# chengstone/cchess-zero

Hardware: AMD Instinct MI355X
Metric: MCTS simulations/sec (whole node), playout=1600, 7-block net (higher is better)
Workload: dtype mx6

## Files before the change

cchess_zero_amd/csrc/cz_trunk_mx.h:

```cpp
#pragma once
#include "cz_conv_kernel.h"

namespace czconv {

#include "cz_trunk_mx_asm.inc"

struct MXGeo {
    static constexpr int P = 2;
    static constexpr int ROWS = P * 90;
    static constexpr int THREADS = 512;
    static constexpr int ENT = 224;
    static constexpr int XPLANE = ENT * 16, YPLANE = ENT * 8, SPLANE = ENT * 4;
    static constexpr int X_OFF = 0, Y_OFF = 8 * XPLANE, S_OFF = Y_OFF + 8 * YPLANE;
    static constexpr int HI_OFF = S_OFF + 2 * SPLANE;
    static constexpr int ZERO_OFF = HI_OFF + ROWS * CV_ROWB;
    static constexpr int W_OFF = ZERO_OFF + CV_ROWB;
    static constexpr int SLAB_BYTES = 16384;
    static constexpr int SLAB_SHIFT = 14;
    static constexpr int SLABS_PER_LAYER = 36;
    static constexpr int LDS_BYTES = W_OFF + TW_NBUF * SLAB_BYTES;
    static constexpr int PLANES_OFF = W_OFF + 3 * SLAB_BYTES;
    static constexpr int HEADW_OFF = LDS_BYTES;
    static constexpr int LDS_TOTAL = LDS_BYTES + 3 * 128 * 4;
    static constexpr int F32_ROWB = 512;
// ... 198 lines not shown
    }

#define MX_OPERANDS(NAB, NKEY)                                                                                       \
            : [c0] "+v"(acc[0]), [c1] "+v"(acc[1]), [c2] "+v"(acc[2]),                                                 \
              [a0h0] "+v"(fa.a[0]), [a0h1] "+v"(fa.a[1]), [a0h2] "+v"(fa.a[2]), [w0] "+v"(fa.w),                      \
              [a1h0] "+v"(fb.a[0]), [a1h1] "+v"(fb.a[1]), [a1h2] "+v"(fb.a[2]), [w1] "+v"(fb.w),                      \
              [sb0] "+v"(sb[0]), [sb1] "+v"(sb[1]), [sb2] "+v"(sb[2]),                                                \
              [t0] "=&v"(t0), [t1] "=&v"(t1), [t2] "=&v"(t2), [ws] "=&v"(wsr), [keep] "=&s"(keep)                      \
            : [ab0] "v"(ab[0]), [ab1] "v"(ab[1]), [ab2] "v"(ab[2]), [key0] "v"(key[0]), [key1] "v"(key[1]),            \
              [key2] "v"(key[2]), [nab0] "v"(NAB[0]), [nab1] "v"(NAB[1]), [nab2] "v"(NAB[2]), [nkey0] "v"(NKEY[0]),     \
              [nkey1] "v"(NKEY[1]), [nkey2] "v"(NKEY[2]), [xr0] "v"(xr[0]), [xr1] "v"(xr[1]), [xr2] "v"(xr[2]),        \
              [yr0] "v"(yr[0]), [yr1] "v"(yr[1]), [yr2] "v"(yr[2]), [vb] "v"(vb), [vy] "v"(vy), [vs] "v"(vs),          \
              [vbn] "v"(vbn), [voff0] "v"(voff0), [voff1] "v"(voff1), [sbase] "s"(sbase), [ldst] "s"(ldst)
#define MX_CLOBBERS "memory", "scc", "v232", "v233", "v234", "v235", "v236", "v237", "v238", "v239", "v240", "v241", "v242", "v243", \
                    "v244", "v245", "v246", "v247", "v248", "v249", "v250", "v251", "v252", "v253", "v254", "v255"
#define MX_ARGS()                                                                                                    \
            TRUNK_SLAB_ARGS(wpk, const int vy = vy0 + slot; const int vs = vs0 + slot;)
#define MX_RUN(ASMSTR, NAB, NKEY)                                                                                    \
        {                                                                                                            \
            MX_ARGS()                                                                                                \
            asm volatile(ASMSTR MX_OPERANDS(NAB, NKEY) : MX_CLOBBERS);                                               \
            ++g;                                                                                                     \
        }
#define MX_RUNV(ASMSTR, NAB, NKEY)                           \
        {                                                                                                            \
            MX_ARGS()                                                                                                \
            asm volatile(ASMSTR MX_OPERANDS(NAB, NKEY), [skipm] "s"(skipm) : MX_CLOBBERS, "vcc");                    \
            ++g;                                                                                                     \
        }

#ifdef MX_TIMING
    unsigned long long tm_loop = 0, tm_epi = 0, tm_set = 0, tm_t0 = __builtin_readcyclecounter();
    const unsigned long long tm_first = tm_t0 - clk_c0;
#define MX_TM(acc) { const unsigned long long n_ = __builtin_readcyclecounter(); acc += n_ - tm_t0; tm_t0 = n_; }
#else
#define MX_TM(acc)
#endif
    struct MxFrag { bf16x8 a[3], w; };
    int g = 0;
    int skipm;
    asm volatile("s_cmp_lt_u32 %1, 4\n\ts_cselect_b32 %0, 1, 0" : "=s"(skipm) : "s"(wave_u) : "scc");
#pragma unroll 1
    for (int layer = 0; layer < nlayers; ++layer) {
        f32x16 acc[3];
        init_acc(acc, nullptr, (layer & 1) != 0);
        int ab[3], key[3], nab[3], nkey[3], xr[3], yr[3], nxr[3], nyr[3], t0, t1, t2, wsr;
        int sb[3] = {0, 0, 0};
        MxFrag fa, fb;
        tap_addr(0, ab, key, xr, yr);
        {
            const int vb = vb0 + (((unsigned)g & 3u) << Geo::SLAB_SHIFT);
#pragma unroll
            for (int i = 0; i < 3; ++i) {
                fa.a[i] = *reinterpret_cast<const bf16x8 *>(smem + ab[i] + ((0 ^ key[i]) << 4));
                fb.a[i] = *reinterpret_cast<const bf16x8 *>(smem + ab[i] + ((2 ^ key[i]) << 4));
            }
            fa.w = *reinterpret_cast<const bf16x8 *>(smem + vb);
            fb.w = *reinterpret_cast<const bf16x8 *>(smem + vb + 4096);
            asm volatile("" : "+v"(fa.a[0]), "+v"(fa.a[1]), "+v"(fa.a[2]), "+v"(fa.w), "+v"(fb.a[0]), "+v"(fb.a[1]), "+v"(fb.a[2]), "+v"(fb.w));
        }
        MX_TM(tm_set)
        int tap = 0;
#pragma unroll 1
        for (; tap < 3; ++tap) {
            MX_RUNV(MX_SKIP0_ASM_Q0, ab, key)
            MX_RUNV(MX_SKIP0_ASM_Q1, ab, key)
            MX_RUNV(MX_SKIP0_ASM_Q2, ab, key)
            tap_addr(tap + 1, nab, nkey, nxr, nyr);
            MX_RUNV(MX_SKIP0_ASM_Q3, nab, nkey)
#pragma unroll
            for (int i = 0; i < 3; ++i) { ab[i] = nab[i]; key[i] = nkey[i]; xr[i] = nxr[i]; yr[i] = nyr[i]; }
        }
#pragma unroll 1
        for (; tap < 8; ++tap) {
            MX_RUN(MX_SLAB_ASM_Q0, ab, key)
            MX_RUN(MX_SLAB_ASM_Q1, ab, key)
            MX_RUN(MX_SLAB_ASM_Q2, ab, key)
            tap_addr(tap + 1, nab, nkey, nxr, nyr);
            MX_RUN(MX_SLAB_ASM_Q3, nab, nkey)
#pragma unroll
            for (int i = 0; i < 3; ++i) { ab[i] = nab[i]; key[i] = nkey[i]; xr[i] = nxr[i]; yr[i] = nyr[i]; }
        }
        MX_RUN(MX_SLAB_ASM_Q0, ab, key)
        MX_RUN(MX_SLAB_ASM_Q1, ab, key)
        MX_RUN(MX_SLAB_ASM_Q2, ab, key)
        MX_RUN(MX_SLAB_ASM_Q3_LAST, ab, key)
        const bool last = layer + 1 == nlayers;
        if (last) asm volatile("s_waitcnt vmcnt(0)" ::: "memory");
        else load_bias(bias + (layer + 1) * 128);
        asm volatile("s_nop 15\n\ts_nop 15\n\ts_nop 15" ::: "memory");
        MX_TM(tm_loop)
        refresh_rk();
// ... 27 lines not shown
        for (int r = tid; r < nrows; r += Geo::THREADS) {
            const int k = lds_row_of(r);
            float acc0 = 0.f, acc1 = 0.f, acc2 = 0.f;
#pragma unroll 4
            for (int c = 0; c < 32; ++c) {
                const float4 e = *reinterpret_cast<const float4 *>(smem + k * Geo::F32_ROWB + ((c ^ (k & 31)) << 4));
                const float *w0_ = hw + c * 4, *w1_ = hw + 128 + c * 4, *w2_ = hw + 256 + c * 4;
                acc0 += e.x * w0_[0] + e.y * w0_[1] + e.z * w0_[2] + e.w * w0_[3];
                acc1 += e.x * w1_[0] + e.y * w1_[1] + e.z * w1_[2] + e.w * w1_[3];
                acc2 += e.x * w2_[0] + e.y * w2_[1] + e.z * w2_[2] + e.w * w2_[3];
            }
            float *o = head_out + ((size_t)pos0 * 90 + r) * 3;
            o[0] = fmaxf(acc0 + head_b[0], 0.f);
            o[1] = fmaxf(acc1 + head_b[1], 0.f);
            o[2] = fmaxf(acc2 + head_b[2], 0.f);
        }
    }
}
#undef MX_OPERANDS
#undef MX_CLOBBERS
#undef MX_ARGS
#undef MX_RUN
#undef MX_RUNV

}
```

cchess_zero_amd/csrc/cz_trunk_mx_asm.inc:

```
#define MX_SLAB_ASM_Q0 \
    "s_mov_b32 %[keep], m0\n\t" \
    "s_waitcnt lgkmcnt(4)\n\t" \
    "v_mfma_f32_32x32x16_f16 %[c0], %[w0], %[a0h0], %[c0]\n\t" \
    "ds_read_b128 v[232:235], %[xr0] offset:0\n\t" \
    "ds_read_b64 v[236:237], %[yr0] offset:28672\n\t" \
    "ds_read_b128 v[238:241], %[xr1] offset:0\n\t" \
    "ds_read_b64 v[242:243], %[yr1] offset:28672\n\t" \
    "v_lshrrev_b32 %[t0], 1, %[yr0]\n\t" \
    "v_lshrrev_b32 %[t1], 1, %[yr1]\n\t" \
    "v_lshrrev_b32 %[t2], 1, %[yr2]\n\t" \
    "v_mfma_f32_32x32x16_f16 %[c1], %[w0], %[a0h1], %[c1]\n\t" \
    "ds_read_b128 v[244:247], %[xr2] offset:0\n\t" \
    "ds_read_b64 v[248:249], %[yr2] offset:28672\n\t" \
    "ds_read_b32 %[sb0], %[t0] offset:43008\n\t" \
    "ds_read_b32 %[sb1], %[t1] offset:43008\n\t" \
    "ds_read_b32 %[sb2], %[t2] offset:43008\n\t" \
    "v_mfma_f32_32x32x16_f16 %[c2], %[w0], %[a0h2], %[c2]\n\t" \
    "ds_read_b128 v[250:253], %[vb] offset:8192\n\t" \
    "ds_read_b64 v[254:255], %[vy]\n\t" \
    "ds_read_b32 %[ws], %[vs]\n\t" \
    "s_waitcnt vmcnt(2)\n\t" \
    "s_barrier\n\t" \
    "s_waitcnt lgkmcnt(12)\n\t" \
    "v_mfma_f32_32x32x16_f16 %[c0], %[w1], %[a1h0], %[c0]\n\t" \
// ... 170 lines not shown
    "ds_read_b128 %[w0], %[vbn]\n\t" \
    "s_waitcnt lgkmcnt(4)\n\t" \
    "v_mfma_scale_f32_32x32x64_f8f6f4 %[c0], v[250:255], v[232:237], %[c0], %[ws], %[sb0] op_sel:[0,1,0] op_sel_hi:[0,1,0] cbsz:2 blgp:2\n\t" \
    "v_xor_b32 %[t0], 2, %[nkey0]\n\t" \
    "v_xor_b32 %[t1], 2, %[nkey1]\n\t" \
    "v_xor_b32 %[t2], 2, %[nkey2]\n\t" \
    "v_lshl_add_u32 %[t0], %[t0], 4, %[nab0]\n\t" \
    "v_lshl_add_u32 %[t1], %[t1], 4, %[nab1]\n\t" \
    "v_lshl_add_u32 %[t2], %[t2], 4, %[nab2]\n\t" \
    "s_mov_b32 m0, %[ldst]\n\t" \
    "s_nop 0\n\t" \
    "global_load_lds_dwordx4 %[voff0], %[sbase]\n\t" \
    "v_mfma_scale_f32_32x32x64_f8f6f4 %[c1], v[250:255], v[238:243], %[c1], %[ws], %[sb1] op_sel:[0,1,0] op_sel_hi:[0,1,0] cbsz:2 blgp:2\n\t" \
    "ds_read_b128 %[a1h0], %[t0]\n\t" \
    "ds_read_b128 %[a1h1], %[t1]\n\t" \
    "s_add_u32 m0, %[ldst], 0x2000\n\t" \
    "s_nop 0\n\t" \
    "global_load_lds_dwordx4 %[voff1], %[sbase]\n\t" \
    "v_mfma_scale_f32_32x32x64_f8f6f4 %[c2], v[250:255], v[244:249], %[c2], %[ws], %[sb2] op_sel:[0,1,0] op_sel_hi:[0,1,0] cbsz:2 blgp:2\n\t" \
    "ds_read_b128 %[a1h2], %[t2]\n\t" \
    "ds_read_b128 %[w1], %[vbn] offset:4096\n\t" \
    "s_mov_b32 m0, %[keep]\n\t"

#define MX_SKIP0_ASM_Q0 \
    "s_cmp_lg_u32 %[skipm], 0\n\t" \
    "s_cselect_b64 vcc, -1, 0\n\t" \
    "s_mov_b32 %[keep], m0\n\t" \
    "s_waitcnt lgkmcnt(4)\n\t" \
    "s_cbranch_vccnz 1f\n\t" \
    "v_mfma_f32_32x32x16_f16 %[c0], %[w0], %[a0h0], %[c0]\n\t" \
    "1:\n\t" \
    "ds_read_b128 v[232:235], %[xr0] offset:0\n\t" \
    "ds_read_b64 v[236:237], %[yr0] offset:28672\n\t" \
    "ds_read_b128 v[238:241], %[xr1] offset:0\n\t" \
    "ds_read_b64 v[242:243], %[yr1] offset:28672\n\t" \
    "v_lshrrev_b32 %[t0], 1, %[yr0]\n\t" \
    "v_lshrrev_b32 %[t1], 1, %[yr1]\n\t" \
    "v_lshrrev_b32 %[t2], 1, %[yr2]\n\t" \
    "v_mfma_f32_32x32x16_f16 %[c1], %[w0], %[a0h1], %[c1]\n\t" \
    "ds_read_b128 v[244:247], %[xr2] offset:0\n\t" \
    "ds_read_b64 v[248:249], %[yr2] offset:28672\n\t" \
    "ds_read_b32 %[sb0], %[t0] offset:43008\n\t" \
    "ds_read_b32 %[sb1], %[t1] offset:43008\n\t" \
    "ds_read_b32 %[sb2], %[t2] offset:43008\n\t" \
    "v_mfma_f32_32x32x16_f16 %[c2], %[w0], %[a0h2], %[c2]\n\t" \
    "ds_read_b128 v[250:253], %[vb] offset:8192\n\t" \
    "ds_read_b64 v[254:255], %[vy]\n\t" \
    "ds_read_b32 %[ws], %[vs]\n\t" \
    "s_waitcnt vmcnt(2)\n\t" \
    "s_barrier\n\t" \
    "s_waitcnt lgkmcnt(12)\n\t" \
    "s_cbranch_vccnz 1f\n\t" \
    "v_mfma_f32_32x32x16_f16 %[c0], %[w1], %[a1h0], %[c0]\n\t" \
    "1:\n\t" \
    "v_xor_b32 %[t0], 4, %[key0]\n\t" \
    "v_xor_b32 %[t1], 4, %[key1]\n\t" \
    "v_xor_b32 %[t2], 4, %[key2]\n\t" \
    "v_lshl_add_u32 %[t0], %[t0], 4, %[ab0]\n\t" \
    "v_lshl_add_u32 %[t1], %[t1], 4, %[ab1]\n\t" \
    "v_lshl_add_u32 %[t2], %[t2], 4, %[ab2]\n\t" \
    "v_mfma_f32_32x32x16_f16 %[c1], %[w1], %[a1h1], %[c1]\n\t" \
    "ds_read_b128 %[a0h0], %[t0]\n\t" \
    "ds_read_b128 %[a0h1], %[t1]\n\t" \
    "v_mfma_f32_32x32x16_f16 %[c2], %[w1], %[a1h2], %[c2]\n\t" \
    "ds_read_b128 %[a0h2], %[t2]\n\t" \
    "ds_read_b128 %[w0], %[vbn]\n\t" \
    "s_waitcnt lgkmcnt(4)\n\t" \
    "s_cbranch_vccnz 1f\n\t" \
    "v_mfma_scale_f32_32x32x64_f8f6f4 %[c0], v[250:255], v[232:237], %[c0], %[ws], %[sb0] op_sel:[0,0,0] op_sel_hi:[0,0,0] cbsz:2 blgp:2\n\t" \
    "1:\n\t" \
    "v_xor_b32 %[t0], 6, %[key0]\n\t" \
    "v_xor_b32 %[t1], 6, %[key1]\n\t" \
    "v_xor_b32 %[t2], 6, %[key2]\n\t" \
    "v_lshl_add_u32 %[t0], %[t0], 4, %[ab0]\n\t" \
    "v_lshl_add_u32 %[t1], %[t1], 4, %[ab1]\n\t" \
    "v_lshl_add_u32 %[t2], %[t2], 4, %[ab2]\n\t" \
    "s_mov_b32 m0, %[ldst]\n\t" \
    "s_nop 0\n\t" \
    "global_load_lds_dwordx4 %[voff0], %[sbase]\n\t" \
    "v_mfma_scale_f32_32x32x64_f8f6f4 %[c1], v[250:255], v[238:243], %[c1], %[ws], %[sb1] op_sel:[0,0,0] op_sel_hi:[0,0,0] cbsz:2 blgp:2\n\t" \
    "ds_read_b128 %[a1h0], %[t0]\n\t" \
    "ds_read_b128 %[a1h1], %[t1]\n\t" \
    "s_add_u32 m0, %[ldst], 0x2000\n\t" \
    "s_nop 0\n\t" \
    "global_load_lds_dwordx4 %[voff1], %[sbase]\n\t" \
    "v_mfma_scale_f32_32x32x64_f8f6f4 %[c2], v[250:255], v[244:249], %[c2], %[ws], %[sb2] op_sel:[0,0,0] op_sel_hi:[0,0,0] cbsz:2 blgp:2\n\t" \
    "ds_read_b128 %[a1h2], %[t2]\n\t" \
    "ds_read_b128 %[w1], %[vbn] offset:4096\n\t" \
    "s_mov_b32 m0, %[keep]\n\t"

#define MX_SKIP0_ASM_Q1 \
    "s_cmp_lg_u32 %[skipm], 0\n\t" \
    "s_cselect_b64 vcc, -1, 0\n\t" \
    "s_mov_b32 %[keep], m0\n\t" \
    "s_waitcnt lgkmcnt(4)\n\t" \
    "s_cbranch_vccnz 1f\n\t" \
    "v_mfma_f32_32x32x16_f16 %[c0], %[w0], %[a0h0], %[c0]\n\t" \
    "1:\n\t" \
    "ds_read_b128 v[232:235], %[xr0] offset:7168\n\t" \
    "ds_read_b64 v[236:237], %[yr0] offset:32256\n\t" \
    "ds_read_b128 v[238:241], %[xr1] offset:7168\n\t" \
    "ds_read_b64 v[242:243], %[yr1] offset:32256\n\t" \
    "v_mfma_f32_32x32x16_f16 %[c1], %[w0], %[a0h1], %[c1]\n\t" \
    "ds_read_b128 v[244:247], %[xr2] offset:7168\n\t" \
    "ds_read_b64 v[248:249], %[yr2] offset:32256\n\t" \
    "v_mfma_f32_32x32x16_f16 %[c2], %[w0], %[a0h2], %[c2]\n\t" \
    "ds_read_b128 v[250:253], %[vb] offset:8192\n\t" \
    "ds_read_b64 v[254:255], %[vy]\n\t" \
    "ds_read_b32 %[ws], %[vs]\n\t" \
    "s_waitcnt vmcnt(2)\n\t" \
    "s_barrier\n\t" \
    "s_waitcnt lgkmcnt(9)\n\t" \
    "s_cbranch_vccnz 1f\n\t" \
    "v_mfma_f32_32x32x16_f16 %[c0], %[w1], %[a1h0], %[c0]\n\t" \
    "1:\n\t" \
    "v_xor_b32 %[t0], 8, %[key0]\n\t" \
    "v_xor_b32 %[t1], 8, %[key1]\n\t" \
    "v_xor_b32 %[t2], 8, %[key2]\n\t" \
    "v_lshl_add_u32 %[t0], %[t0], 4, %[ab0]\n\t" \
    "v_lshl_add_u32 %[t1], %[t1], 4, %[ab1]\n\t" \
    "v_lshl_add_u32 %[t2], %[t2], 4, %[ab2]\n\t" \
    "v_mfma_f32_32x32x16_f16 %[c1], %[w1], %[a1h1], %[c1]\n\t" \
    "ds_read_b128 %[a0h0], %[t0]\n\t" \
    "ds_read_b128 %[a0h1], %[t1]\n\t" \
    "v_mfma_f32_32x32x16_f16 %[c2], %[w1], %[a1h2], %[c2]\n\t" \
    "ds_read_b128 %[a0h2], %[t2]\n\t" \
    "ds_read_b128 %[w0], %[vbn]\n\t" \
    "s_waitcnt lgkmcnt(4)\n\t" \
    "s_cbranch_vccnz 1f\n\t" \
    "v_mfma_scale_f32_32x32x64_f8f6f4 %[c0], v[250:255], v[232:237], %[c0], %[ws], %[sb0] op_sel:[0,1,0] op_sel_hi:[0,0,0] cbsz:2 blgp:2\n\t" \
    "1:\n\t" \
    "v_xor_b32 %[t0], 10, %[key0]\n\t" \
    "v_xor_b32 %[t1], 10, %[key1]\n\t" \
    "v_xor_b32 %[t2], 10, %[key2]\n\t" \
    "v_lshl_add_u32 %[t0], %[t0], 4, %[ab0]\n\t" \
    "v_lshl_add_u32 %[t1], %[t1], 4, %[ab1]\n\t" \
    "v_lshl_add_u32 %[t2], %[t2], 4, %[ab2]\n\t" \
    "s_mov_b32 m0, %[ldst]\n\t" \
    "s_nop 0\n\t" \
    "global_load_lds_dwordx4 %[voff0], %[sbase]\n\t" \
    "v_mfma_scale_f32_32x32x64_f8f6f4 %[c1], v[250:255], v[238:243], %[c1], %[ws], %[sb1] op_sel:[0,1,0] op_sel_hi:[0,0,0] cbsz:2 blgp:2\n\t" \
    "ds_read_b128 %[a1h0], %[t0]\n\t" \
    "ds_read_b128 %[a1h1], %[t1]\n\t" \
    "s_add_u32 m0, %[ldst], 0x2000\n\t" \
    "s_nop 0\n\t" \
    "global_load_lds_dwordx4 %[voff1], %[sbase]\n\t" \
    "v_mfma_scale_f32_32x32x64_f8f6f4 %[c2], v[250:255], v[244:249], %[c2], %[ws], %[sb2] op_sel:[0,1,0] op_sel_hi:[0,0,0] cbsz:2 blgp:2\n\t" \
    "ds_read_b128 %[a1h2], %[t2]\n\t" \
    "ds_read_b128 %[w1], %[vbn] offset:4096\n\t" \
    "s_mov_b32 m0, %[keep]\n\t"

#define MX_SKIP0_ASM_Q2 \
    "s_cmp_lg_u32 %[skipm], 0\n\t" \
    "s_cselect_b64 vcc, -1, 0\n\t" \
    "s_mov_b32 %[keep], m0\n\t" \
    "s_waitcnt lgkmcnt(4)\n\t" \
    "s_cbranch_vccnz 1f\n\t" \
    "v_mfma_f32_32x32x16_f16 %[c0], %[w0], %[a0h0], %[c0]\n\t" \
    "1:\n\t" \
    "ds_read_b128 v[232:235], %[xr0] offset:14336\n\t" \
    "ds_read_b64 v[236:237], %[yr0] offset:35840\n\t" \
    "ds_read_b128 v[238:241], %[xr1] offset:14336\n\t" \
    "ds_read_b64 v[242:243], %[yr1] offset:35840\n\t" \
    "v_mfma_f32_32x32x16_f16 %[c1], %[w0], %[a0h1], %[c1]\n\t" \
    "ds_read_b128 v[244:247], %[xr2] offset:14336\n\t" \
    "ds_read_b64 v[248:249], %[yr2] offset:35840\n\t" \
    "v_mfma_f32_32x32x16_f16 %[c2], %[w0], %[a0h2], %[c2]\n\t" \
    "ds_read_b128 v[250:253], %[vb] offset:8192\n\t" \
    "ds_read_b64 v[254:255], %[vy]\n\t" \
    "ds_read_b32 %[ws], %[vs]\n\t" \
    "s_waitcnt vmcnt(2)\n\t" \
    "s_barrier\n\t" \
    "s_waitcnt lgkmcnt(9)\n\t" \
    "s_cbranch_vccnz 1f\n\t" \
    "v_mfma_f32_32x32x16_f16 %[c0], %[w1], %[a1h0], %[c0]\n\t" \
    "1:\n\t" \
    "v_xor_b32 %[t0], 12, %[key0]\n\t" \
    "v_xor_b32 %[t1], 12, %[key1]\n\t" \
    "v_xor_b32 %[t2], 12, %[key2]\n\t" \
    "v_lshl_add_u32 %[t0], %[t0], 4, %[ab0]\n\t" \
    "v_lshl_add_u32 %[t1], %[t1], 4, %[ab1]\n\t" \
    "v_lshl_add_u32 %[t2], %[t2], 4, %[ab2]\n\t" \
    "v_mfma_f32_32x32x16_f16 %[c1], %[w1], %[a1h1], %[c1]\n\t" \
    "ds_read_b128 %[a0h0], %[t0]\n\t" \
    "ds_read_b128 %[a0h1], %[t1]\n\t" \
    "v_mfma_f32_32x32x16_f16 %[c2], %[w1], %[a1h2], %[c2]\n\t" \
    "ds_read_b128 %[a0h2], %[t2]\n\t" \
    "ds_read_b128 %[w0], %[vbn]\n\t" \
    "s_waitcnt lgkmcnt(4)\n\t" \
    "s_cbranch_vccnz 1f\n\t" \
    "v_mfma_scale_f32_32x32x64_f8f6f4 %[c0], v[250:255], v[232:237], %[c0], %[ws], %[sb0] op_sel:[0,0,0] op_sel_hi:[0,1,0] cbsz:2 blgp:2\n\t" \
    "1:\n\t" \
    "v_xor_b32 %[t0], 14, %[key0]\n\t" \
    "v_xor_b32 %[t1], 14, %[key1]\n\t" \
    "v_xor_b32 %[t2], 14, %[key2]\n\t" \
    "v_lshl_add_u32 %[t0], %[t0], 4, %[ab0]\n\t" \
    "v_lshl_add_u32 %[t1], %[t1], 4, %[ab1]\n\t" \
    "v_lshl_add_u32 %[t2], %[t2], 4, %[ab2]\n\t" \
    "s_mov_b32 m0, %[ldst]\n\t" \
    "s_nop 0\n\t" \
    "global_load_lds_dwordx4 %[voff0], %[sbase]\n\t" \
    "v_mfma_scale_f32_32x32x64_f8f6f4 %[c1], v[250:255], v[238:243], %[c1], %[ws], %[sb1] op_sel:[0,0,0] op_sel_hi:[0,1,0] cbsz:2 blgp:2\n\t" \
    "ds_read_b128 %[a1h0], %[t0]\n\t" \
    "ds_read_b128 %[a1h1], %[t1]\n\t" \
    "s_add_u32 m0, %[ldst], 0x2000\n\t" \
    "s_nop 0\n\t" \
    "global_load_lds_dwordx4 %[voff1], %[sbase]\n\t" \
    "v_mfma_scale_f32_32x32x64_f8f6f4 %[c2], v[250:255], v[244:249], %[c2], %[ws], %[sb2] op_sel:[0,0,0] op_sel_hi:[0,1,0] cbsz:2 blgp:2\n\t" \
    "ds_read_b128 %[a1h2], %[t2]\n\t" \
    "ds_read_b128 %[w1], %[vbn] offset:4096\n\t" \
    "s_mov_b32 m0, %[keep]\n\t"

#define MX_SKIP0_ASM_Q3 \
    "s_cmp_lg_u32 %[skipm], 0\n\t" \
    "s_cselect_b64 vcc, -1, 0\n\t" \
    "s_mov_b32 %[keep], m0\n\t" \
    "s_waitcnt lgkmcnt(4)\n\t" \
    "s_cbranch_vccnz 1f\n\t" \
    "v_mfma_f32_32x32x16_f16 %[c0], %[w0], %[a0h0], %[c0]\n\t" \
    "1:\n\t" \
    "ds_read_b128 v[232:235], %[xr0] offset:21504\n\t" \
    "ds_read_b64 v[236:237], %[yr0] offset:39424\n\t" \
    "ds_read_b128 v[238:241], %[xr1] offset:21504\n\t" \
    "ds_read_b64 v[242:243], %[yr1] offset:39424\n\t" \
    "v_mfma_f32_32x32x16_f16 %[c1], %[w0], %[a0h1], %[c1]\n\t" \
    "ds_read_b128 v[244:247], %[xr2] offset:21504\n\t" \
    "ds_read_b64 v[248:249], %[yr2] offset:39424\n\t" \
    "v_mfma_f32_32x32x16_f16 %[c2], %[w0], %[a0h2], %[c2]\n\t" \
    "ds_read_b128 v[250:253], %[vb] offset:8192\n\t" \
    "ds_read_b64 v[254:255], %[vy]\n\t" \
    "ds_read_b32 %[ws], %[vs]\n\t" \
    "s_waitcnt vmcnt(2)\n\t" \
    "s_barrier\n\t" \
    "s_waitcnt lgkmcnt(9)\n\t" \
    "s_cbranch_vccnz 1f\n\t" \
    "v_mfma_f32_32x32x16_f16 %[c0], %[w1], %[a1h0], %[c0]\n\t" \
    "1:\n\t" \
    "v_xor_b32 %[t0], 0, %[nkey0]\n\t" \
    "v_xor_b32 %[t1], 0, %[nkey1]\n\t" \
    "v_xor_b32 %[t2], 0, %[nkey2]\n\t" \
    "v_lshl_add_u32 %[t0], %[t0], 4, %[nab0]\n\t" \
    "v_lshl_add_u32 %[t1], %[t1], 4, %[nab1]\n\t" \
    "v_lshl_add_u32 %[t2], %[t2], 4, %[nab2]\n\t" \
    "v_mfma_f32_32x32x16_f16 %[c1], %[w1], %[a1h1], %[c1]\n\t" \
    "ds_read_b128 %[a0h0], %[t0]\n\t" \
    "ds_read_b128 %[a0h1], %[t1]\n\t" \
    "v_mfma_f32_32x32x16_f16 %[c2], %[w1], %[a1h2], %[c2]\n\t" \
    "ds_read_b128 %[a0h2], %[t2]\n\t" \
    "ds_read_b128 %[w0], %[vbn]\n\t" \
    "s_waitcnt lgkmcnt(4)\n\t" \
    "s_cbranch_vccnz 1f\n\t" \
    "v_mfma_scale_f32_32x32x64_f8f6f4 %[c0], v[250:255], v[232:237], %[c0], %[ws], %[sb0] op_sel:[0,1,0] op_sel_hi:[0,1,0] cbsz:2 blgp:2\n\t" \
    "1:\n\t" \
    "v_xor_b32 %[t0], 2, %[nkey0]\n\t" \
    "v_xor_b32 %[t1], 2, %[nkey1]\n\t" \
    "v_xor_b32 %[t2], 2, %[nkey2]\n\t" \
    "v_lshl_add_u32 %[t0], %[t0], 4, %[nab0]\n\t" \
    "v_lshl_add_u32 %[t1], %[t1], 4, %[nab1]\n\t" \
    "v_lshl_add_u32 %[t2], %[t2], 4, %[nab2]\n\t" \
    "s_mov_b32 m0, %[ldst]\n\t" \
    "s_nop 0\n\t" \
    "global_load_lds_dwordx4 %[voff0], %[sbase]\n\t" \
    "v_mfma_scale_f32_32x32x64_f8f6f4 %[c1], v[250:255], v[238:243], %[c1], %[ws], %[sb1] op_sel:[0,1,0] op_sel_hi:[0,1,0] cbsz:2 blgp:2\n\t" \
    "ds_read_b128 %[a1h0], %[t0]\n\t" \
    "ds_read_b128 %[a1h1], %[t1]\n\t" \
    "s_add_u32 m0, %[ldst], 0x2000\n\t" \
    "s_nop 0\n\t" \
    "global_load_lds_dwordx4 %[voff1], %[sbase]\n\t" \
    "v_mfma_scale_f32_32x32x64_f8f6f4 %[c2], v[250:255], v[244:249], %[c2], %[ws], %[sb2] op_sel:[0,1,0] op_sel_hi:[0,1,0] cbsz:2 blgp:2\n\t" \
    "ds_read_b128 %[a1h2], %[t2]\n\t" \
    "ds_read_b128 %[w1], %[vbn] offset:4096\n\t" \
    "s_mov_b32 m0, %[keep]\n\t"

#define MX_SLAB_ASM_Q3_LAST \
    "s_mov_b32 %[keep], m0\n\t" \
    "s_waitcnt lgkmcnt(4)\n\t" \
    "v_mfma_f32_32x32x16_f16 %[c0], %[w0], %[a0h0], %[c0]\n\t" \
    "ds_read_b128 v[232:235], %[xr0] offset:21504\n\t" \
    "ds_read_b64 v[236:237], %[yr0] offset:39424\n\t" \
    "ds_read_b128 v[238:241], %[xr1] offset:21504\n\t" \
    "ds_read_b64 v[242:243], %[yr1] offset:39424\n\t" \
    "v_mfma_f32_32x32x16_f16 %[c1], %[w0], %[a0h1], %[c1]\n\t" \
    "ds_read_b128 v[244:247], %[xr2] offset:21504\n\t" \
    "ds_read_b64 v[248:249], %[yr2] offset:39424\n\t" \
    "v_mfma_f32_32x32x16_f16 %[c2], %[w0], %[a0h2], %[c2]\n\t" \
    "ds_read_b128 v[250:253], %[vb] offset:8192\n\t" \
    "ds_read_b64 v[254:255], %[vy]\n\t" \
    "ds_read_b32 %[ws], %[vs]\n\t" \
    "s_waitcnt vmcnt(2) lgkmcnt(0)\n\t" \
    "s_barrier\n\t" \
    "v_mfma_f32_32x32x16_f16 %[c0], %[w1], %[a1h0], %[c0]\n\t" \
    "v_mfma_f32_32x32x16_f16 %[c1], %[w1], %[a1h1], %[c1]\n\t" \
    "v_mfma_f32_32x32x16_f16 %[c2], %[w1], %[a1h2], %[c2]\n\t" \
    "v_mfma_scale_f32_32x32x64_f8f6f4 %[c0], v[250:255], v[232:237], %[c0], %[ws], %[sb0] op_sel:[0,1,0] op_sel_hi:[0,1,0] cbsz:2 blgp:2\n\t" \
    "s_mov_b32 m0, %[ldst]\n\t" \
// ... 10 lines not shown
```

Before: 2.000 million.

## Specialize skip-tap path for low waves to drop dead row-0 loads and MFMAs

Replaces the per-instruction vcc-branch skipping of the c0 MFMAs for waves below 4 with separate asm variants selected once per quarter-slab. The low-wave variants omit the row-0 MFMAs, their LDS reads (x/y/scale) and the tap address math, with lgkmcnt waits adjusted to the smaller number of outstanding reads. A special next-tap Q3 variant restores the full preload when leaving the skip region. This adds scalar branch dispatch, code size and fragile hand-counted waitcnts in exchange for fewer LDS reads and branches on the skip waves.

```diff
diff --git a/cchess_zero_amd/csrc/cz_trunk_mx.h b/cchess_zero_amd/csrc/cz_trunk_mx.h
--- a/cchess_zero_amd/csrc/cz_trunk_mx.h
+++ b/cchess_zero_amd/csrc/cz_trunk_mx.h
@@ -244,10 +244,14 @@
             asm volatile(ASMSTR MX_OPERANDS(NAB, NKEY) : MX_CLOBBERS);                                               \
             ++g;                                                                                                     \
         }
-#define MX_RUNV(ASMSTR, NAB, NKEY)                           \
+#define MX_DY(G0, PLAIN) "s_cmp_eq_u32 %[sel], 0\n\ts_cbranch_scc1 3f\n\t" G0 "s_branch 4f\n\t3:\n\t" PLAIN "4:\n\t"
+#define MX_DY3(G0, G0N, PLAIN)                                                                                       \
+        "s_cmp_eq_u32 %[sel], 0\n\ts_cbranch_scc1 3f\n\ts_cmp_eq_u32 %[sel], 1\n\ts_cbranch_scc1 5f\n\t"                \
+        G0N "s_branch 4f\n\t5:\n\t" G0 "s_branch 4f\n\t3:\n\t" PLAIN "4:\n\t"
+#define MX_RUNV(ASMSTR, NAB, NKEY, SEL)                                   \
         {                                                                                                            \
             MX_ARGS()                                                                                                \
-            asm volatile(ASMSTR MX_OPERANDS(NAB, NKEY), [skipm] "s"(skipm) : MX_CLOBBERS, "vcc");                    \
+            asm volatile(ASMSTR MX_OPERANDS(NAB, NKEY), [sel] "s"(SEL) : MX_CLOBBERS);                                \
             ++g;                                                                                                     \
         }
 
@@ -260,8 +264,8 @@
 #endif
     struct MxFrag { bf16x8 a[3], w; };
     int g = 0;
-    int skipm;
-    asm volatile("s_cmp_lt_u32 %1, 4\n\ts_cselect_b32 %0, 1, 0" : "=s"(skipm) : "s"(wave_u) : "scc");
+    int g0;
+    asm volatile("s_cmp_lt_u32 %1, 4\n\ts_cselect_b32 %0, 1, 0" : "=s"(g0) : "s"(wave_u) : "scc");
 #pragma unroll 1
     for (int layer = 0; layer < nlayers; ++layer) {
         f32x16 acc[3];
@@ -272,24 +276,25 @@
         tap_addr(0, ab, key, xr, yr);
         {
             const int vb = vb0 + (((unsigned)g & 3u) << Geo::SLAB_SHIFT);
-#pragma unroll
-            for (int i = 0; i < 3; ++i) {
-                fa.a[i] = *reinterpret_cast<const bf16x8 *>(smem + ab[i] + ((0 ^ key[i]) << 4));
-                fb.a[i] = *reinterpret_cast<const bf16x8 *>(smem + ab[i] + ((2 ^ key[i]) << 4));
-            }
-            fa.w = *reinterpret_cast<const bf16x8 *>(smem + vb);
-            fb.w = *reinterpret_cast<const bf16x8 *>(smem + vb + 4096);
-            asm volatile("" : "+v"(fa.a[0]), "+v"(fa.a[1]), "+v"(fa.a[2]), "+v"(fa.w), "+v"(fb.a[0]), "+v"(fb.a[1]), "+v"(fb.a[2]), "+v"(fb.w));
+            asm volatile(MX_DY(MX_G0_PRELOAD_ASM, MX_PRELOAD_ASM)
+                         : [a0h0] "=&v"(fa.a[0]), [a0h1] "=&v"(fa.a[1]), [a0h2] "=&v"(fa.a[2]), [w0] "=&v"(fa.w),
+                           [a1h0] "=&v"(fb.a[0]), [a1h1] "=&v"(fb.a[1]), [a1h2] "=&v"(fb.a[2]), [w1] "=&v"(fb.w),
+                           [t0] "=&v"(t0), [t1] "=&v"(t1), [t2] "=&v"(t2)
+                         : [ab0] "v"(ab[0]), [ab1] "v"(ab[1]), [ab2] "v"(ab[2]), [key0] "v"(key[0]), [key1] "v"(key[1]),
+                           [key2] "v"(key[2]), [vb] "v"(vb), [sel] "s"(g0)
+                         : "memory", "scc");
         }
         MX_TM(tm_set)
         int tap = 0;
 #pragma unroll 1
         for (; tap < 3; ++tap) {
-            MX_RUNV(MX_SKIP0_ASM_Q0, ab, key)
-            MX_RUNV(MX_SKIP0_ASM_Q1, ab, key)
-            MX_RUNV(MX_SKIP0_ASM_Q2, ab, key)
+            MX_RUNV(MX_DY(MX_G0_ASM_Q0, MX_SLAB_ASM_Q0), ab, key, g0)
+            MX_RUNV(MX_DY(MX_G0_ASM_Q1, MX_SLAB_ASM_Q1), ab, key, g0)
+            MX_RUNV(MX_DY(MX_G0_ASM_Q2, MX_SLAB_ASM_Q2), ab, key, g0)
             tap_addr(tap + 1, nab, nkey, nxr, nyr);
-            MX_RUNV(MX_SKIP0_ASM_Q3, nab, nkey)
+            int sel3;
+            asm("s_lshl_b32 %0, %1, %2" : "=s"(sel3) : "s"(g0), "s"(tap >> 1) : "scc");
+            MX_RUNV(MX_DY3(MX_G0_ASM_Q3, MX_G0_ASM_Q3_NEXT, MX_SLAB_ASM_Q3), nab, nkey, sel3)
 #pragma unroll
             for (int i = 0; i < 3; ++i) { ab[i] = nab[i]; key[i] = nkey[i]; xr[i] = nxr[i]; yr[i] = nyr[i]; }
         }
@@ -363,5 +368,7 @@
 #undef MX_ARGS
 #undef MX_RUN
 #undef MX_RUNV
+#undef MX_DY
+#undef MX_DY3
 
 }
diff --git a/cchess_zero_amd/csrc/cz_trunk_mx_asm.inc b/cchess_zero_amd/csrc/cz_trunk_mx_asm.inc
--- a/cchess_zero_amd/csrc/cz_trunk_mx_asm.inc
+++ b/cchess_zero_amd/csrc/cz_trunk_mx_asm.inc
@@ -216,64 +216,65 @@
     "ds_read_b128 %[w1], %[vbn] offset:4096\n\t" \
     "s_mov_b32 m0, %[keep]\n\t"
 
-#define MX_SKIP0_ASM_Q0 \
-    "s_cmp_lg_u32 %[skipm], 0\n\t" \
-    "s_cselect_b64 vcc, -1, 0\n\t" \
-    "s_mov_b32 %[keep], m0\n\t" \
-    "s_waitcnt lgkmcnt(4)\n\t" \
-    "s_cbranch_vccnz 1f\n\t" \
-    "v_mfma_f32_32x32x16_f16 %[c0], %[w0], %[a0h0], %[c0]\n\t" \
-    "1:\n\t" \
-    "ds_read_b128 v[232:235], %[xr0] offset:0\n\t" \
-    "ds_read_b64 v[236:237], %[yr0] offset:28672\n\t" \
+#define MX_PRELOAD_ASM \
+    "v_xor_b32 %[t0], 0, %[key0]\n\t" \
+    "v_xor_b32 %[t1], 0, %[key1]\n\t" \
+    "v_xor_b32 %[t2], 0, %[key2]\n\t" \
+    "v_lshl_add_u32 %[t0], %[t0], 4, %[ab0]\n\t" \
+    "v_lshl_add_u32 %[t1], %[t1], 4, %[ab1]\n\t" \
+    "v_lshl_add_u32 %[t2], %[t2], 4, %[ab2]\n\t" \
+    "ds_read_b128 %[a0h0], %[t0]\n\t" \
+    "ds_read_b128 %[a0h1], %[t1]\n\t" \
+    "ds_read_b128 %[a0h2], %[t2]\n\t" \
+    "ds_read_b128 %[w0], %[vb]\n\t" \
+    "v_xor_b32 %[t0], 2, %[key0]\n\t" \
+    "v_xor_b32 %[t1], 2, %[key1]\n\t" \
+    "v_xor_b32 %[t2], 2, %[key2]\n\t" \
+    "v_lshl_add_u32 %[t0], %[t0], 4, %[ab0]\n\t" \
+    "v_lshl_add_u32 %[t1], %[t1], 4, %[ab1]\n\t" \
+    "v_lshl_add_u32 %[t2], %[t2], 4, %[ab2]\n\t" \
+    "ds_read_b128 %[a1h0], %[t0]\n\t" \
+    "ds_read_b128 %[a1h1], %[t1]\n\t" \
+    "ds_read_b128 %[a1h2], %[t2]\n\t" \
+    "ds_read_b128 %[w1], %[vb] offset:4096\n\t"
+
+#define MX_G0_ASM_Q0 \
+    "s_mov_b32 %[keep], m0\n\t" \
+    "s_waitcnt lgkmcnt(3)\n\t" \
+    "v_mfma_f32_32x32x16_f16 %[c1], %[w0], %[a0h1], %[c1]\n\t" \
     "ds_read_b128 v[238:241], %[xr1] offset:0\n\t" \
     "ds_read_b64 v[242:243], %[yr1] offset:28672\n\t" \
-    "v_lshrrev_b32 %[t0], 1, %[yr0]\n\t" \
+    "ds_read_b128 v[244:247], %[xr2] offset:0\n\t" \
+    "ds_read_b64 v[248:249], %[yr2] offset:28672\n\t" \
     "v_lshrrev_b32 %[t1], 1, %[yr1]\n\t" \
     "v_lshrrev_b32 %[t2], 1, %[yr2]\n\t" \
-    "v_mfma_f32_32x32x16_f16 %[c1], %[w0], %[a0h1], %[c1]\n\t" \
-    "ds_read_b128 v[244:247], %[xr2] offset:0\n\t" \
-    "ds_read_b64 v[248:249], %[yr2] offset:28672\n\t" \
-    "ds_read_b32 %[sb0], %[t0] offset:43008\n\t" \
+    "v_mfma_f32_32x32x16_f16 %[c2], %[w0], %[a0h2], %[c2]\n\t" \
     "ds_read_b32 %[sb1], %[t1] offset:43008\n\t" \
     "ds_read_b32 %[sb2], %[t2] offset:43008\n\t" \
-    "v_mfma_f32_32x32x16_f16 %[c2], %[w0], %[a0h2], %[c2]\n\t" \
-    "ds_read_b128 v[250:253], %[vb] offset:8192\n\t" \
-    "ds_read_b64 v[254:255], %[vy]\n\t" \
-    "ds_read_b32 %[ws], %[vs]\n\t" \
-    "s_waitcnt vmcnt(2)\n\t" \
-    "s_barrier\n\t" \
-    "s_waitcnt lgkmcnt(12)\n\t" \
-    "s_cbranch_vccnz 1f\n\t" \
-    "v_mfma_f32_32x32x16_f16 %[c0], %[w1], %[a1h0], %[c0]\n\t" \
-    "1:\n\t" \
-    "v_xor_b32 %[t0], 4, %[key0]\n\t" \
+    "ds_read_b128 v[250:253], %[vb] offset:8192\n\t" \
+    "ds_read_b64 v[254:255], %[vy]\n\t" \
+    "ds_read_b32 %[ws], %[vs]\n\t" \
+    "s_waitcnt vmcnt(2)\n\t" \
+    "s_barrier\n\t" \
+    "s_waitcnt lgkmcnt(9)\n\t" \
+    "v_mfma_f32_32x32x16_f16 %[c1], %[w1], %[a1h1], %[c1]\n\t" \
     "v_xor_b32 %[t1], 4, %[key1]\n\t" \
     "v_xor_b32 %[t2], 4, %[key2]\n\t" \
-    "v_lshl_add_u32 %[t0], %[t0], 4, %[ab0]\n\t" \
-    "v_lshl_add_u32 %[t1], %[t1], 4, %[ab1]\n\t" \
-    "v_lshl_add_u32 %[t2], %[t2], 4, %[ab2]\n\t" \
-    "v_mfma_f32_32x32x16_f16 %[c1], %[w1], %[a1h1], %[c1]\n\t" \
-    "ds_read_b128 %[a0h0], %[t0]\n\t" \
-    "ds_read_b128 %[a0h1], %[t1]\n\t" \
-    "v_mfma_f32_32x32x16_f16 %[c2], %[w1], %[a1h2], %[c2]\n\t" \
-    "ds_read_b128 %[a0h2], %[t2]\n\t" \
-    "ds_read_b128 %[w0], %[vbn]\n\t" \
-    "s_waitcnt lgkmcnt(4)\n\t" \
-    "s_cbranch_vccnz 1f\n\t" \
-    "v_mfma_scale_f32_32x32x64_f8f6f4 %[c0], v[250:255], v[232:237], %[c0], %[ws], %[sb0] op_sel:[0,0,0] op_sel_hi:[0,0,0] cbsz:2 blgp:2\n\t" \
-    "1:\n\t" \
-    "v_xor_b32 %[t0], 6, %[key0]\n\t" \
+    "v_lshl_add_u32 %[t1], %[t1], 4, %[ab1]\n\t" \
+    "v_lshl_add_u32 %[t2], %[t2], 4, %[ab2]\n\t" \
+    "ds_read_b128 %[a0h1], %[t1]\n\t" \
+    "v_mfma_f32_32x32x16_f16 %[c2], %[w1], %[a1h2], %[c2]\n\t" \
+    "ds_read_b128 %[a0h2], %[t2]\n\t" \
+    "ds_read_b128 %[w0], %[vbn]\n\t" \
+    "s_waitcnt lgkmcnt(3)\n\t" \
+    "v_mfma_scale_f32_32x32x64_f8f6f4 %[c1], v[250:255], v[238:243], %[c1], %[ws], %[sb1] op_sel:[0,0,0] op_sel_hi:[0,0,0] cbsz:2 blgp:2\n\t" \
     "v_xor_b32 %[t1], 6, %[key1]\n\t" \
     "v_xor_b32 %[t2], 6, %[key2]\n\t" \
-    "v_lshl_add_u32 %[t0], %[t0], 4, %[ab0]\n\t" \
-    "v_lshl_add_u32 %[t1], %[t1], 4, %[ab1]\n\t" \
-    "v_lshl_add_u32 %[t2], %[t2], 4, %[ab2]\n\t" \
-    "s_mov_b32 m0, %[ldst]\n\t" \
-    "s_nop 0\n\t" \
-    "global_load_lds_dwordx4 %[voff0], %[sbase]\n\t" \
-    "v_mfma_scale_f32_32x32x64_f8f6f4 %[c1], v[250:255], v[238:243], %[c1], %[ws], %[sb1] op_sel:[0,0,0] op_sel_hi:[0,0,0] cbsz:2 blgp:2\n\t" \
-    "ds_read_b128 %[a1h0], %[t0]\n\t" \
+    "v_lshl_add_u32 %[t1], %[t1], 4, %[ab1]\n\t" \
+    "v_lshl_add_u32 %[t2], %[t2], 4, %[ab2]\n\t" \
+    "s_mov_b32 m0, %[ldst]\n\t" \
+    "s_nop 0\n\t" \
+    "global_load_lds_dwordx4 %[voff0], %[sbase]\n\t" \
     "ds_read_b128 %[a1h1], %[t1]\n\t" \
     "s_add_u32 m0, %[ldst], 0x2000\n\t" \
     "s_nop 0\n\t" \
@@ -283,19 +284,12 @@
     "ds_read_b128 %[w1], %[vbn] offset:4096\n\t" \
     "s_mov_b32 m0, %[keep]\n\t"
 
-#define MX_SKIP0_ASM_Q1 \
-    "s_cmp_lg_u32 %[skipm], 0\n\t" \
-    "s_cselect_b64 vcc, -1, 0\n\t" \
-    "s_mov_b32 %[keep], m0\n\t" \
-    "s_waitcnt lgkmcnt(4)\n\t" \
-    "s_cbranch_vccnz 1f\n\t" \
-    "v_mfma_f32_32x32x16_f16 %[c0], %[w0], %[a0h0], %[c0]\n\t" \
-    "1:\n\t" \
-    "ds_read_b128 v[232:235], %[xr0] offset:7168\n\t" \
-    "ds_read_b64 v[236:237], %[yr0] offset:32256\n\t" \
+#define MX_G0_ASM_Q1 \
+    "s_mov_b32 %[keep], m0\n\t" \
+    "s_waitcnt lgkmcnt(3)\n\t" \
+    "v_mfma_f32_32x32x16_f16 %[c1], %[w0], %[a0h1], %[c1]\n\t" \
     "ds_read_b128 v[238:241], %[xr1] offset:7168\n\t" \
     "ds_read_b64 v[242:243], %[yr1] offset:32256\n\t" \
-    "v_mfma_f32_32x32x16_f16 %[c1], %[w0], %[a0h1], %[c1]\n\t" \
     "ds_read_b128 v[244:247], %[xr2] offset:7168\n\t" \
     "ds_read_b64 v[248:249], %[yr2] offset:32256\n\t" \
     "v_mfma_f32_32x32x16_f16 %[c2], %[w0], %[a0h2], %[c2]\n\t" \
@@ -304,37 +298,25 @@
     "ds_read_b32 %[ws], %[vs]\n\t" \
     "s_waitcnt vmcnt(2)\n\t" \
     "s_barrier\n\t" \
-    "s_waitcnt lgkmcnt(9)\n\t" \
-    "s_cbranch_vccnz 1f\n\t" \
-    "v_mfma_f32_32x32x16_f16 %[c0], %[w1], %[a1h0], %[c0]\n\t" \
-    "1:\n\t" \
-    "v_xor_b32 %[t0], 8, %[key0]\n\t" \
+    "s_waitcnt lgkmcnt(7)\n\t" \
+    "v_mfma_f32_32x32x16_f16 %[c1], %[w1], %[a1h1], %[c1]\n\t" \
     "v_xor_b32 %[t1], 8, %[key1]\n\t" \
     "v_xor_b32 %[t2], 8, %[key2]\n\t" \
-    "v_lshl_add_u32 %[t0], %[t0], 4, %[ab0]\n\t" \
-    "v_lshl_add_u32 %[t1], %[t1], 4, %[ab1]\n\t" \
-    "v_lshl_add_u32 %[t2], %[t2], 4, %[ab2]\n\t" \
-    "v_mfma_f32_32x32x16_f16 %[c1], %[w1], %[a1h1], %[c1]\n\t" \
-    "ds_read_b128 %[a0h0], %[t0]\n\t" \
-    "ds_read_b128 %[a0h1], %[t1]\n\t" \
-    "v_mfma_f32_32x32x16_f16 %[c2], %[w1], %[a1h2], %[c2]\n\t" \
-    "ds_read_b128 %[a0h2], %[t2]\n\t" \
-    "ds_read_b128 %[w0], %[vbn]\n\t" \
-    "s_waitcnt lgkmcnt(4)\n\t" \
-    "s_cbranch_vccnz 1f\n\t" \
-    "v_mfma_scale_f32_32x32x64_f8f6f4 %[c0], v[250:255], v[232:237], %[c0], %[ws], %[sb0] op_sel:[0,1,0] op_sel_hi:[0,0,0] cbsz:2 blgp:2\n\t" \
-    "1:\n\t" \
-    "v_xor_b32 %[t0], 10, %[key0]\n\t" \
+    "v_lshl_add_u32 %[t1], %[t1], 4, %[ab1]\n\t" \
+    "v_lshl_add_u32 %[t2], %[t2], 4, %[ab2]\n\t" \
+    "ds_read_b128 %[a0h1], %[t1]\n\t" \
+    "v_mfma_f32_32x32x16_f16 %[c2], %[w1], %[a1h2], %[c2]\n\t" \
+    "ds_read_b128 %[a0h2], %[t2]\n\t" \
+    "ds_read_b128 %[w0], %[vbn]\n\t" \
+    "s_waitcnt lgkmcnt(3)\n\t" \
+    "v_mfma_scale_f32_32x32x64_f8f6f4 %[c1], v[250:255], v[238:243], %[c1], %[ws], %[sb1] op_sel:[0,1,0] op_sel_hi:[0,0,0] cbsz:2 blgp:2\n\t" \
     "v_xor_b32 %[t1], 10, %[key1]\n\t" \
     "v_xor_b32 %[t2], 10, %[key2]\n\t" \
-    "v_lshl_add_u32 %[t0], %[t0], 4, %[ab0]\n\t" \
-    "v_lshl_add_u32 %[t1], %[t1], 4, %[ab1]\n\t" \
-    "v_lshl_add_u32 %[t2], %[t2], 4, %[ab2]\n\t" \
-    "s_mov_b32 m0, %[ldst]\n\t" \
-    "s_nop 0\n\t" \
-    "global_load_lds_dwordx4 %[voff0], %[sbase]\n\t" \
-    "v_mfma_scale_f32_32x32x64_f8f6f4 %[c1], v[250:255], v[238:243], %[c1], %[ws], %[sb1] op_sel:[0,1,0] op_sel_hi:[0,0,0] cbsz:2 blgp:2\n\t" \
-    "ds_read_b128 %[a1h0], %[t0]\n\t" \
+    "v_lshl_add_u32 %[t1], %[t1], 4, %[ab1]\n\t" \
+    "v_lshl_add_u32 %[t2], %[t2], 4, %[ab2]\n\t" \
+    "s_mov_b32 m0, %[ldst]\n\t" \
+    "s_nop 0\n\t" \
+    "global_load_lds_dwordx4 %[voff0], %[sbase]\n\t" \
     "ds_read_b128 %[a1h1], %[t1]\n\t" \
     "s_add_u32 m0, %[ldst], 0x2000\n\t" \
     "s_nop 0\n\t" \
@@ -344,19 +326,12 @@
     "ds_read_b128 %[w1], %[vbn] offset:4096\n\t" \
     "s_mov_b32 m0, %[keep]\n\t"
 
-#define MX_SKIP0_ASM_Q2 \
-    "s_cmp_lg_u32 %[skipm], 0\n\t" \
-    "s_cselect_b64 vcc, -1, 0\n\t" \
-    "s_mov_b32 %[keep], m0\n\t" \
-    "s_waitcnt lgkmcnt(4)\n\t" \
-    "s_cbranch_vccnz 1f\n\t" \
-    "v_mfma_f32_32x32x16_f16 %[c0], %[w0], %[a0h0], %[c0]\n\t" \
-    "1:\n\t" \
-    "ds_read_b128 v[232:235], %[xr0] offset:14336\n\t" \
-    "ds_read_b64 v[236:237], %[yr0] offset:35840\n\t" \
+#define MX_G0_ASM_Q2 \
+    "s_mov_b32 %[keep], m0\n\t" \
+    "s_waitcnt lgkmcnt(3)\n\t" \
+    "v_mfma_f32_32x32x16_f16 %[c1], %[w0], %[a0h1], %[c1]\n\t" \
     "ds_read_b128 v[238:241], %[xr1] offset:14336\n\t" \
     "ds_read_b64 v[242:243], %[yr1] offset:35840\n\t" \
-    "v_mfma_f32_32x32x16_f16 %[c1], %[w0], %[a0h1], %[c1]\n\t" \
     "ds_read_b128 v[244:247], %[xr2] offset:14336\n\t" \
     "ds_read_b64 v[248:249], %[yr2] offset:35840\n\t" \
     "v_mfma_f32_32x32x16_f16 %[c2], %[w0], %[a0h2], %[c2]\n\t" \
@@ -365,37 +340,25 @@
     "ds_read_b32 %[ws], %[vs]\n\t" \
     "s_waitcnt vmcnt(2)\n\t" \
     "s_barrier\n\t" \
-    "s_waitcnt lgkmcnt(9)\n\t" \
-    "s_cbranch_vccnz 1f\n\t" \
-    "v_mfma_f32_32x32x16_f16 %[c0], %[w1], %[a1h0], %[c0]\n\t" \
-    "1:\n\t" \
-    "v_xor_b32 %[t0], 12, %[key0]\n\t" \
+    "s_waitcnt lgkmcnt(7)\n\t" \
+    "v_mfma_f32_32x32x16_f16 %[c1], %[w1], %[a1h1], %[c1]\n\t" \
     "v_xor_b32 %[t1], 12, %[key1]\n\t" \
     "v_xor_b32 %[t2], 12, %[key2]\n\t" \
-    "v_lshl_add_u32 %[t0], %[t0], 4, %[ab0]\n\t" \
-    "v_lshl_add_u32 %[t1], %[t1], 4, %[ab1]\n\t" \
-    "v_lshl_add_u32 %[t2], %[t2], 4, %[ab2]\n\t" \
-    "v_mfma_f32_32x32x16_f16 %[c1], %[w1], %[a1h1], %[c1]\n\t" \
-    "ds_read_b128 %[a0h0], %[t0]\n\t" \
-    "ds_read_b128 %[a0h1], %[t1]\n\t" \
-    "v_mfma_f32_32x32x16_f16 %[c2], %[w1], %[a1h2], %[c2]\n\t" \
-    "ds_read_b128 %[a0h2], %[t2]\n\t" \
-    "ds_read_b128 %[w0], %[vbn]\n\t" \
-    "s_waitcnt lgkmcnt(4)\n\t" \
-    "s_cbranch_vccnz 1f\n\t" \
-    "v_mfma_scale_f32_32x32x64_f8f6f4 %[c0], v[250:255], v[232:237], %[c0], %[ws], %[sb0] op_sel:[0,0,0] op_sel_hi:[0,1,0] cbsz:2 blgp:2\n\t" \
-    "1:\n\t" \
-    "v_xor_b32 %[t0], 14, %[key0]\n\t" \
+    "v_lshl_add_u32 %[t1], %[t1], 4, %[ab1]\n\t" \
+    "v_lshl_add_u32 %[t2], %[t2], 4, %[ab2]\n\t" \
+    "ds_read_b128 %[a0h1], %[t1]\n\t" \
+    "v_mfma_f32_32x32x16_f16 %[c2], %[w1], %[a1h2], %[c2]\n\t" \
+    "ds_read_b128 %[a0h2], %[t2]\n\t" \
+    "ds_read_b128 %[w0], %[vbn]\n\t" \
+    "s_waitcnt lgkmcnt(3)\n\t" \
+    "v_mfma_scale_f32_32x32x64_f8f6f4 %[c1], v[250:255], v[238:243], %[c1], %[ws], %[sb1] op_sel:[0,0,0] op_sel_hi:[0,1,0] cbsz:2 blgp:2\n\t" \
     "v_xor_b32 %[t1], 14, %[key1]\n\t" \
     "v_xor_b32 %[t2], 14, %[key2]\n\t" \
-    "v_lshl_add_u32 %[t0], %[t0], 4, %[ab0]\n\t" \
-    "v_lshl_add_u32 %[t1], %[t1], 4, %[ab1]\n\t" \
-    "v_lshl_add_u32 %[t2], %[t2], 4, %[ab2]\n\t" \
-    "s_mov_b32 m0, %[ldst]\n\t" \
-    "s_nop 0\n\t" \
-    "global_load_lds_dwordx4 %[voff0], %[sbase]\n\t" \
-    "v_mfma_scale_f32_32x32x64_f8f6f4 %[c1], v[250:255], v[238:243], %[c1], %[ws], %[sb1] op_sel:[0,0,0] op_sel_hi:[0,1,0] cbsz:2 blgp:2\n\t" \
-    "ds_read_b128 %[a1h0], %[t0]\n\t" \
+    "v_lshl_add_u32 %[t1], %[t1], 4, %[ab1]\n\t" \
+    "v_lshl_add_u32 %[t2], %[t2], 4, %[ab2]\n\t" \
+    "s_mov_b32 m0, %[ldst]\n\t" \
+    "s_nop 0\n\t" \
+    "global_load_lds_dwordx4 %[voff0], %[sbase]\n\t" \
     "ds_read_b128 %[a1h1], %[t1]\n\t" \
     "s_add_u32 m0, %[ldst], 0x2000\n\t" \
     "s_nop 0\n\t" \
@@ -405,19 +368,12 @@
     "ds_read_b128 %[w1], %[vbn] offset:4096\n\t" \
     "s_mov_b32 m0, %[keep]\n\t"
 
-#define MX_SKIP0_ASM_Q3 \
-    "s_cmp_lg_u32 %[skipm], 0\n\t" \
-    "s_cselect_b64 vcc, -1, 0\n\t" \
-    "s_mov_b32 %[keep], m0\n\t" \
-    "s_waitcnt lgkmcnt(4)\n\t" \
-    "s_cbranch_vccnz 1f\n\t" \
-    "v_mfma_f32_32x32x16_f16 %[c0], %[w0], %[a0h0], %[c0]\n\t" \
-    "1:\n\t" \
-    "ds_read_b128 v[232:235], %[xr0] offset:21504\n\t" \
-    "ds_read_b64 v[236:237], %[yr0] offset:39424\n\t" \
+#define MX_G0_ASM_Q3 \
+    "s_mov_b32 %[keep], m0\n\t" \
+    "s_waitcnt lgkmcnt(3)\n\t" \
+    "v_mfma_f32_32x32x16_f16 %[c1], %[w0], %[a0h1], %[c1]\n\t" \
     "ds_read_b128 v[238:241], %[xr1] offset:21504\n\t" \
     "ds_read_b64 v[242:243], %[yr1] offset:39424\n\t" \
-    "v_mfma_f32_32x32x16_f16 %[c1], %[w0], %[a0h1], %[c1]\n\t" \
     "ds_read_b128 v[244:247], %[xr2] offset:21504\n\t" \
     "ds_read_b64 v[248:249], %[yr2] offset:39424\n\t" \
     "v_mfma_f32_32x32x16_f16 %[c2], %[w0], %[a0h2], %[c2]\n\t" \
@@ -426,26 +382,63 @@
     "ds_read_b32 %[ws], %[vs]\n\t" \
     "s_waitcnt vmcnt(2)\n\t" \
     "s_barrier\n\t" \
-    "s_waitcnt lgkmcnt(9)\n\t" \
-    "s_cbranch_vccnz 1f\n\t" \
-    "v_mfma_f32_32x32x16_f16 %[c0], %[w1], %[a1h0], %[c0]\n\t" \
-    "1:\n\t" \
+    "s_waitcnt lgkmcnt(7)\n\t" \
+    "v_mfma_f32_32x32x16_f16 %[c1], %[w1], %[a1h1], %[c1]\n\t" \
+    "v_xor_b32 %[t1], 0, %[nkey1]\n\t" \
+    "v_xor_b32 %[t2], 0, %[nkey2]\n\t" \
+    "v_lshl_add_u32 %[t1], %[t1], 4, %[nab1]\n\t" \
+    "v_lshl_add_u32 %[t2], %[t2], 4, %[nab2]\n\t" \
+    "ds_read_b128 %[a0h1], %[t1]\n\t" \
+    "v_mfma_f32_32x32x16_f16 %[c2], %[w1], %[a1h2], %[c2]\n\t" \
+    "ds_read_b128 %[a0h2], %[t2]\n\t" \
+    "ds_read_b128 %[w0], %[vbn]\n\t" \
+    "s_waitcnt lgkmcnt(3)\n\t" \
+    "v_mfma_scale_f32_32x32x64_f8f6f4 %[c1], v[250:255], v[238:243], %[c1], %[ws], %[sb1] op_sel:[0,1,0] op_sel_hi:[0,1,0] cbsz:2 blgp:2\n\t" \
+    "v_xor_b32 %[t1], 2, %[nkey1]\n\t" \
+    "v_xor_b32 %[t2], 2, %[nkey2]\n\t" \
+    "v_lshl_add_u32 %[t1], %[t1], 4, %[nab1]\n\t" \
+    "v_lshl_add_u32 %[t2], %[t2], 4, %[nab2]\n\t" \
+    "s_mov_b32 m0, %[ldst]\n\t" \
+    "s_nop 0\n\t" \
+    "global_load_lds_dwordx4 %[voff0], %[sbase]\n\t" \
+    "ds_read_b128 %[a1h1], %[t1]\n\t" \
+    "s_add_u32 m0, %[ldst], 0x2000\n\t" \
+    "s_nop 0\n\t" \
+    "global_load_lds_dwordx4 %[voff1], %[sbase]\n\t" \
+    "v_mfma_scale_f32_32x32x64_f8f6f4 %[c2], v[250:255], v[244:249], %[c2], %[ws], %[sb2] op_sel:[0,1,0] op_sel_hi:[0,1,0] cbsz:2 blgp:2\n\t" \
+    "ds_read_b128 %[a1h2], %[t2]\n\t" \
+    "ds_read_b128 %[w1], %[vbn] offset:4096\n\t" \
+    "s_mov_b32 m0, %[keep]\n\t"
+
+#define MX_G0_ASM_Q3_NEXT \
+    "s_mov_b32 %[keep], m0\n\t" \
+    "s_waitcnt lgkmcnt(3)\n\t" \
+    "v_mfma_f32_32x32x16_f16 %[c1], %[w0], %[a0h1], %[c1]\n\t" \
+    "ds_read_b128 v[238:241], %[xr1] offset:21504\n\t" \
+    "ds_read_b64 v[242:243], %[yr1] offset:39424\n\t" \
+    "ds_read_b128 v[244:247], %[xr2] offset:21504\n\t" \
+    "ds_read_b64 v[248:249], %[yr2] offset:39424\n\t" \
+    "v_mfma_f32_32x32x16_f16 %[c2], %[w0], %[a0h2], %[c2]\n\t" \
+    "ds_read_b128 v[250:253], %[vb] offset:8192\n\t" \
+    "ds_read_b64 v[254:255], %[vy]\n\t" \
+    "ds_read_b32 %[ws], %[vs]\n\t" \
+    "s_waitcnt vmcnt(2)\n\t" \
+    "s_barrier\n\t" \
+    "s_waitcnt lgkmcnt(7)\n\t" \
+    "v_mfma_f32_32x32x16_f16 %[c1], %[w1], %[a1h1], %[c1]\n\t" \
     "v_xor_b32 %[t0], 0, %[nkey0]\n\t" \
     "v_xor_b32 %[t1], 0, %[nkey1]\n\t" \
     "v_xor_b32 %[t2], 0, %[nkey2]\n\t" \
     "v_lshl_add_u32 %[t0], %[t0], 4, %[nab0]\n\t" \
     "v_lshl_add_u32 %[t1], %[t1], 4, %[nab1]\n\t" \
     "v_lshl_add_u32 %[t2], %[t2], 4, %[nab2]\n\t" \
-    "v_mfma_f32_32x32x16_f16 %[c1], %[w1], %[a1h1], %[c1]\n\t" \
     "ds_read_b128 %[a0h0], %[t0]\n\t" \
     "ds_read_b128 %[a0h1], %[t1]\n\t" \
     "v_mfma_f32_32x32x16_f16 %[c2], %[w1], %[a1h2], %[c2]\n\t" \
     "ds_read_b128 %[a0h2], %[t2]\n\t" \
     "ds_read_b128 %[w0], %[vbn]\n\t" \
     "s_waitcnt lgkmcnt(4)\n\t" \
-    "s_cbranch_vccnz 1f\n\t" \
-    "v_mfma_scale_f32_32x32x64_f8f6f4 %[c0], v[250:255], v[232:237], %[c0], %[ws], %[sb0] op_sel:[0,1,0] op_sel_hi:[0,1,0] cbsz:2 blgp:2\n\t" \
-    "1:\n\t" \
+    "v_mfma_scale_f32_32x32x64_f8f6f4 %[c1], v[250:255], v[238:243], %[c1], %[ws], %[sb1] op_sel:[0,1,0] op_sel_hi:[0,1,0] cbsz:2 blgp:2\n\t" \
     "v_xor_b32 %[t0], 2, %[nkey0]\n\t" \
     "v_xor_b32 %[t1], 2, %[nkey1]\n\t" \
     "v_xor_b32 %[t2], 2, %[nkey2]\n\t" \
@@ -455,7 +448,6 @@
     "s_mov_b32 m0, %[ldst]\n\t" \
     "s_nop 0\n\t" \
     "global_load_lds_dwordx4 %[voff0], %[sbase]\n\t" \
-    "v_mfma_scale_f32_32x32x64_f8f6f4 %[c1], v[250:255], v[238:243], %[c1], %[ws], %[sb1] op_sel:[0,1,0] op_sel_hi:[0,1,0] cbsz:2 blgp:2\n\t" \
     "ds_read_b128 %[a1h0], %[t0]\n\t" \
     "ds_read_b128 %[a1h1], %[t1]\n\t" \
     "s_add_u32 m0, %[ldst], 0x2000\n\t" \
@@ -465,6 +457,22 @@
     "ds_read_b128 %[a1h2], %[t2]\n\t" \
     "ds_read_b128 %[w1], %[vbn] offset:4096\n\t" \
     "s_mov_b32 m0, %[keep]\n\t"
+
+#define MX_G0_PRELOAD_ASM \
+    "v_xor_b32 %[t1], 0, %[key1]\n\t" \
+    "v_xor_b32 %[t2], 0, %[key2]\n\t" \
+    "v_lshl_add_u32 %[t1], %[t1], 4, %[ab1]\n\t" \
+    "v_lshl_add_u32 %[t2], %[t2], 4, %[ab2]\n\t" \
+    "ds_read_b128 %[a0h1], %[t1]\n\t" \
+    "ds_read_b128 %[a0h2], %[t2]\n\t" \
+    "ds_read_b128 %[w0], %[vb]\n\t" \
+    "v_xor_b32 %[t1], 2, %[key1]\n\t" \
+    "v_xor_b32 %[t2], 2, %[key2]\n\t" \
+    "v_lshl_add_u32 %[t1], %[t1], 4, %[ab1]\n\t" \
+    "v_lshl_add_u32 %[t2], %[t2], 4, %[ab2]\n\t" \
+    "ds_read_b128 %[a1h1], %[t1]\n\t" \
+    "ds_read_b128 %[a1h2], %[t2]\n\t" \
+    "ds_read_b128 %[w1], %[vb] offset:4096\n\t"
 
 #define MX_SLAB_ASM_Q3_LAST \
     "s_mov_b32 %[keep], m0\n\t" \
```

Result: no change. 1.992 million (-0.4%).
